# MMAThijssen/catfish

Measured on AMD Instinct MI355X. Metric: signal samples/s classified, higher is better.
Workload: dtype f32

## Files before the change

catfish_amd/csrc/catfish_hip.hip:

```cpp
#include <hip/hip_runtime.h>
#include <stdint.h>
#include <string.h>
#include <stdio.h>
#include <vector>
#include <string>
#include <cmath>
#include <mutex>
#include <set>
#include <functional>

#include "../../include/catfish_hip.h"

typedef float f32x4 __attribute__((ext_vector_type(4)));
typedef float f32x2 __attribute__((ext_vector_type(2)));

#define CF_T 35
#define CF_H 64
#define CF_C 32
#define CF_TILE 16

#define MFMA16(a, b, c) __builtin_amdgcn_mfma_f32_16x16x4f32((a), (b), (c), 0, 0, 0)

#ifndef CF_ABLATE
#define CF_ABLATE 0
// ... 52 lines not shown
__device__ __forceinline__ uint32_t cf_fmix32(uint32_t v) {
    v ^= v >> 16; v *= 0x85ebca6bu; v ^= v >> 13; v *= 0xc2b2ae35u; v ^= v >> 16;
    return v;
}
__device__ __forceinline__ uint32_t cf_drop_key(const cf_dropout& d) {
    const uint32_t st = d.step ? (uint32_t)(long long)d.step[0] : 0u;
    return cf_fmix32(d.seed ^ cf_fmix32(0x9E3779B9u * (uint32_t)(d.layer + 1) + st * 0x85ebca6bu));
}
__device__ __forceinline__ f32x4 cf_drop_scale4(uint32_t key, float keep_prob, int64_t idx4) {
    const uint32_t thresh = (uint32_t)fminf(keep_prob * 4294967296.0f, 4294967040.0f);
    const float inv = 1.0f / keep_prob;
    const uint64_t e = (uint64_t)idx4 * 4u;
    const uint32_t base = (uint32_t)e ^ ((uint32_t)(e >> 32) * 0x9E3779B9u);
    f32x4 o;
    o.x = cf_fmix32((base + 0u) ^ key) < thresh ? inv : 0.f;
    o.y = cf_fmix32((base + 1u) ^ key) < thresh ? inv : 0.f;
    o.z = cf_fmix32((base + 2u) ^ key) < thresh ? inv : 0.f;
    o.w = cf_fmix32((base + 3u) ^ key) < thresh ? inv : 0.f;
    return o;
}

__device__ __forceinline__ f32x4 relu4(f32x4 v) {
    f32x4 o;
    o.x = fmaxf(v.x, 0.f); o.y = fmaxf(v.y, 0.f); o.z = fmaxf(v.z, 0.f); o.w = fmaxf(v.w, 0.f);
    return o;
}

__host__ __device__ constexpr int gru_x_floats(int cin) { return (cin / 4) * 3 * 256; }
__host__ __device__ constexpr int gru_hg_floats() { return 16 * 2 * 256; }
__host__ __device__ constexpr int gru_hc_floats() { return 16 * 256; }
__host__ __device__ constexpr int gru_bias_off(int cin) { return gru_x_floats(cin) + gru_hg_floats() + gru_hc_floats(); }
__host__ __device__ constexpr int gru_dense_off(int cin) { return gru_bias_off(cin) + 192; }
__host__ __device__ constexpr int gru_pack_floats(int cin) { return gru_dense_off(cin) + 64; }

__host__ __device__ constexpr int res_units(bool first) { return first ? 4 : 6; }
__host__ __device__ constexpr int res_vecs(bool first) { return first ? 6 : 4; }
__host__ __device__ constexpr int res_pack_floats(bool first) { return res_units(first) * 1024 + res_vecs(first) * 32; }

__host__ __device__ constexpr int frag_feature(int ks, int q) { return 16 * (ks >> 2) + 4 * q + (ks & 3); }

__device__ __forceinline__ void unit_mma(const float* __restrict__ unit, int lane, const f32x4 (&in)[2], f32x4 (&acc)[2]) {
    const f32x2* u2 = reinterpret_cast<const f32x2*>(unit) + lane;
#pragma unroll
    for (int ks = 0; ks < 8; ++ks) {
        const f32x2 a = u2[ks * 64];
        const float b = in[ks >> 2][ks & 3];
        acc[0] = MFMA16(a.x, b, acc[0]);
        acc[1] = MFMA16(a.y, b, acc[1]);
    }
}

template <bool FIRST>
__global__ __launch_bounds__(256) void res_block_kernel(const float* __restrict__ wpack,
                                                        const float* __restrict__ x_nat,
                                                        const f32x4* __restrict__ x_frag,
                                                        f32x4* __restrict__ y_frag,
                                                        int64_t n_windows, int n_tiles, int t_chunks) {
    extern __shared__ __attribute__((aligned(16))) float lds[];
    constexpr int PACK = res_pack_floats(FIRST);
    constexpr int VEC0 = res_units(FIRST) * 1024;
    {
        const f32x4* src = reinterpret_cast<const f32x4*>(wpack);
        f32x4* dst = reinterpret_cast<f32x4*>(lds);
        for (int i = threadIdx.x; i < PACK / 4; i += blockDim.x) dst[i] = src[i];
    }
    __syncthreads();
// ... 168 lines not shown
            }
#pragma unroll
            for (int mo = 0; mo < 2; ++mo) {
                a_pp[mo] = a_p[mo]; a_p[mo] = a_c[mo]; a_sp[mo] = a_sc[mo];
                if (i >= 1) { b_pp[mo] = b_p[mo]; b_p[mo] = b_c[mo]; b_sp[mo] = b_sc[mo]; }
            }
        }
        __builtin_amdgcn_wave_barrier();
    }
}

template <int CIN>
__device__ __forceinline__ void gru_stage_weights(float* lds, const float* __restrict__ wpack, int dir) {
    constexpr int PACK = gru_pack_floats(CIN);
    const f32x4* src = reinterpret_cast<const f32x4*>(wpack + (size_t)dir * PACK);
    f32x4* dst = reinterpret_cast<f32x4*>(lds);
    for (int i = threadIdx.x; i < PACK / 4; i += blockDim.x) dst[i] = src[i];
}

#ifndef CF_SCHED_DS_FIRST
#define CF_SCHED_DS_FIRST 1
#endif
#if CF_SCHED_DS_FIRST
#define CF_KSTEP_SCHED(nds, nmfma)                               \
    __builtin_amdgcn_sched_group_barrier(0x100, nds, 0);         \
    __builtin_amdgcn_sched_group_barrier(0x008, nmfma, 0);       \
    __builtin_amdgcn_sched_barrier(0)
#else
#define CF_KSTEP_SCHED(nds, nmfma) __builtin_amdgcn_sched_barrier(0)
#endif
template <int CIN, bool LAST, bool STASH = false>
__device__ __forceinline__ void gru_tile(const float* lds, int lane, int dir, int tile, const f32x4* __restrict__ X,
                                         f32x4* __restrict__ Y, float* __restrict__ P, int n_tiles,
                                         f32x4* __restrict__ S = nullptr, f32x4* __restrict__ YD = nullptr, cf_dropout drop = cf_dropout()) {
    const uint32_t drop_key = (STASH && YD) ? cf_drop_key(drop) : 0u;
    constexpr int KGX = CIN / 16;
    constexpr int KSX = CIN / 4;
    constexpr int XN4 = gru_x_floats(CIN) / 4;
    constexpr int HG4 = gru_hg_floats() / 4;
    constexpr int BIAS = gru_bias_off(CIN);
    constexpr int DENSE = gru_dense_off(CIN);
    const int q = lane >> 4;
    const f32x4* WX = reinterpret_cast<const f32x4*>(lds) + lane;
    const far_lds<f32x4> WL(WX);
    const f32x4* B4 = reinterpret_cast<const f32x4*>(lds + BIAS) + q;
    const f32x4* D4 = reinterpret_cast<const f32x4*>(lds + DENSE) + q;
    {
        f32x4 h[4] = {{0, 0, 0, 0}, {0, 0, 0, 0}, {0, 0, 0, 0}, {0, 0, 0, 0}};
        f32x4 xc[KGX];
        {
            const int t0 = dir ? (CF_T - 1) : 0;
            const f32x4* src = X + ((int64_t)tile * CF_T + t0) * KGX * 64 + lane;
#pragma unroll
            for (int g = 0; g < KGX; ++g) xc[g] = src[g * 64];
        }
        for (int s = 0; s < CF_T; ++s) {
            const int t = dir ? (CF_T - 1 - s) : s;
            f32x4 acc[12];
#pragma unroll
            for (int mo = 0; mo < 12; ++mo) acc[mo] = B4[mo * 4];
            constexpr int PF = CF_PREFETCH;
            auto loadA = [&](int p, f32x4 (&d)[3]) {
                if (p < KSX) { d[0] = WL[(p * 3 + 0) * 64]; d[1] = WL[(p * 3 + 1) * 64]; d[2] = WL[(p * 3 + 2) * 64]; }
                else if (p < KSX + 16) { d[0] = WL[XN4 + ((p - KSX) * 2 + 0) * 64]; d[1] = WL[XN4 + ((p - KSX) * 2 + 1) * 64]; }
                else if (p < KSX + 32) { d[0] = WL[XN4 + HG4 + (p - KSX - 16) * 64]; }
            };
            f32x4 ac[3], an[3], a2[3];
            loadA(0, ac);
            if (PF == 2) loadA(1, an);
#pragma unroll
            for (int ks = 0; ks < KSX; ++ks) {
                if (PF == 2) loadA(ks + 2, a2); else loadA(ks + 1, an);
                const float b = xc[ks >> 2][ks & 3];
#pragma unroll
                for (int g = 0; g < 3; ++g) {
                    acc[4 * g + 0] = MFMA16(ac[g].x, b, acc[4 * g + 0]);
                    acc[4 * g + 1] = MFMA16(ac[g].y, b, acc[4 * g + 1]);
                    acc[4 * g + 2] = MFMA16(ac[g].z, b, acc[4 * g + 2]);
                    acc[4 * g + 3] = MFMA16(ac[g].w, b, acc[4 * g + 3]);
                }
                CF_KSTEP_SCHED(3, 12);
#pragma unroll
                for (int g = 0; g < 3; ++g) { ac[g] = an[g]; if (PF == 2) an[g] = a2[g]; }
            }
            {
                int tn = dir ? (t - 1) : (t + 1);
                tn = tn < 0 ? 0 : (tn > CF_T - 1 ? CF_T - 1 : tn);
                const f32x4* src = X + ((int64_t)tile * CF_T + tn) * KGX * 64 + lane;
#pragma unroll
// ... 43 lines not shown
                if constexpr (STASH) { acc[4 + m] = u; acc[8 + m] = c; }
            }
            if constexpr (STASH) {
                f32x4* sdst = S + (((int64_t)tile * CF_T + t) * 2 + dir) * 12 * 64 + lane;
#pragma unroll
                for (int j = 0; j < 12; ++j) sdst[j * 64] = acc[j];
            }
            if constexpr (!LAST) {
                f32x4* dst = Y + (((int64_t)tile * CF_T + t) * 8 + dir * 4) * 64 + lane;
#pragma unroll
                for (int m = 0; m < 4; ++m) if (!(CF_ABLATE & 2) || s == CF_T - 1) dst[m * 64] = h[m];
                if constexpr (STASH) {
                    if (YD) {
                        const int64_t i0 = (((int64_t)tile * CF_T + t) * 8 + dir * 4) * 64 + lane;
#pragma unroll
                        for (int m = 0; m < 4; ++m) YD[i0 + m * 64] = h[m] * cf_drop_scale4(drop_key, drop.keep_prob, i0 + m * 64);
                    }
                }
            } else {
                float pm[4];
#pragma unroll
                for (int m = 0; m < 4; ++m) {
                    const f32x4 wd = D4[m * 4];
                    pm[m] = wd.x * h[m].x;
                    pm[m] = fmaf(wd.y, h[m].y, pm[m]); pm[m] = fmaf(wd.z, h[m].z, pm[m]); pm[m] = fmaf(wd.w, h[m].w, pm[m]);
                }
                float p = ((pm[0] + pm[1]) + pm[2]) + pm[3];
                p += __shfl_xor(p, 16);
                p += __shfl_xor(p, 32);
                if (lane < 16) P[(((int64_t)dir * n_tiles + tile) * CF_T + t) * 16 + lane] = p;
            }
            __builtin_amdgcn_sched_barrier(0);
        }
    }
}

template <int CIN, bool LAST>
__global__ __launch_bounds__(512, 2) void gru_layer_kernel(const float* __restrict__ wpack,
                                                           const f32x4* __restrict__ X,
                                                           f32x4* __restrict__ Y,
                                                           float* __restrict__ P,
                                                           int n_tiles) {
    extern __shared__ __attribute__((aligned(16))) float lds[];
    const int dir = blockIdx.y;
    gru_stage_weights<CIN>(lds, wpack, dir);
    __syncthreads();
    const int lane = threadIdx.x & 63;
    const int wave = __builtin_amdgcn_readfirstlane(threadIdx.x >> 6);
    const int nwaves = blockDim.x >> 6;
    const int t0 = (int)((int64_t)blockIdx.x * n_tiles / gridDim.x);
    const int t1 = (int)((int64_t)(blockIdx.x + 1) * n_tiles / gridDim.x);
    for (int tile = t0 + wave; tile < t1; tile += nwaves)
        gru_tile<CIN, LAST>(lds, lane, dir, tile, X, Y, P, n_tiles);
}

struct cf_fused_args {
    const float* w[3];
    const f32x4* x0;
    f32x4* y[2];
    float* p;
    unsigned* flags;
    int lds_floats;
    unsigned* err;
    int n_tiles;
    int groups;
    int n_layers;
    int cin0;
};

__device__ __forceinline__ bool cf_wait_flag(unsigned* flag) {
    for (int it = 0; it < 1000000; ++it) {
        if (__hip_atomic_load(flag, __ATOMIC_RELAXED, __HIP_MEMORY_SCOPE_AGENT) != 0u) return true;
        __builtin_amdgcn_s_sleep(16);
    }
    return false;
}

template <int CIN, bool LAST>
__device__ __forceinline__ void gru_fused_worker(float* lds, const cf_fused_args& a, int layer, int dir) {
    const f32x4* X = layer == 0 ? a.x0 : a.y[(layer - 1) & 1];
    f32x4* Y = a.y[layer & 1];
    gru_stage_weights<CIN>(lds, a.w[layer], dir);
    volatile int* slot = reinterpret_cast<volatile int*>(lds + a.lds_floats);
    unsigned* queue = a.flags + (size_t)a.n_layers * a.groups * 2 + layer * 2 + dir;
    const int lane = threadIdx.x & 63;
    const int wave = __builtin_amdgcn_readfirstlane(threadIdx.x >> 6);
// ... 270 lines not shown
    do {                                                                                           \
        hipError_t e_ = (expr);                                                                    \
        if (e_ != hipSuccess)                                                                      \
            return fail(CF_ERR_HIP, std::string(#expr) + ": " + hipGetErrorString(e_));           \
    } while (0)

enum { SLOT_RES_FIRST = 0, SLOT_RES, SLOT_GRU0, SLOT_GRU, SLOT_GRU_LAST, SLOT_HEAD, SLOT_POST, SLOT_NORM, SLOT_GRU_FUSED, SLOT_RES_STACK2 };
static const char* k_slot_names[CF_PROF_SLOTS] = {"res_block_first", "res_block",      "gru_layer_first", "gru_layer_mid",
                                                  "gru_layer_last",  "head",           "postprocess",     "normalize",       "gru_fused",
                                                  "res_stack2",      "unused",         "unused"};

struct cf_param_map;
static void pm_destroy(cf_param_map* pm);

struct cf_model {
    cf_hparams hp;
    int device = 0;
    int n_cu = 256;
    std::vector<float*> d_res;
    std::vector<float*> d_gru;
    std::vector<int> gru_cin;
    std::vector<char*> d_res_b;
    std::vector<char*> d_gru_b;
    int np = 0;
    float* d_dense_bias = nullptr;
    cf_param_map* pmap = nullptr;
    int64_t cap_windows = 0;
    int64_t cap_tiles = 0;
    struct Slot {
        float* d_a[2] = {nullptr, nullptr};
        float* d_y[2] = {nullptr, nullptr};
        float* d_p = nullptr;
        unsigned* d_flags = nullptr;
        hipStream_t stream = nullptr;
        hipEvent_t done = nullptr;
        int64_t last_windows = 0;
        bool last_res_fused = false;
    };
    std::vector<Slot> slots;
    cf_generic* gen = nullptr;
    int fuse = 0;
    float* d_xp = nullptr;
    int xp_tiles = 0;
    float* d_host_x = nullptr;
    float* d_host_p = nullptr;
    size_t host_stage_bytes = 0;
    unsigned* h_err = nullptr;
    unsigned* d_err = nullptr;
    hipEvent_t fork = nullptr;
    int64_t ws_bytes = 0;
    bool prof = false;
    int prof_every = 0;
    int64_t prof_calls = 0;
    struct Ev { hipEvent_t a, b; int slot; };
    std::vector<Ev> ev_pending;
    std::vector<hipEvent_t> ev_pool;
    double prof_ms[CF_PROF_SLOTS] = {0};
    int64_t prof_n[CF_PROF_SLOTS] = {0};
};

enum { CF_TERM_ZERO = 0, CF_TERM_RAW = 1, CF_TERM_KERN = 2, CF_TERM_BIAS = 3 };
enum { CF_K_ONE = 0, CF_K_GATE = 1, CF_K_CAND = 2 };
__host__ __device__ inline double cf_term_const(int c) { return c == CF_K_GATE ? CF_GATE_SCALE : (c == CF_K_CAND ? CF_CAND_SCALE : 1.0); }

__host__ __device__ inline double cf_bn_scale(float gamma, float var, float eps) {
#pragma clang fp contract(off)
// ... 207 lines not shown
    const size_t pd = off + gru_dense_off(cin);
    for (int i = 0; i < CF_H; ++i) e(pd + i, dense_t >= 0 ? cf_raw(dense_t, dense_e + i) : cf_zero());
}

static void pack_gru_dir(const cf_gru_dir& g, int cin, int cin_real, const float* dense_w ,
                         float* out) {
    cf_host_params P;
    P.t = {g.gates_kernel, g.gates_bias, g.candidate_kernel, g.candidate_bias, dense_w};
    HostSink e{P, out};
    pack_gru_dir(e, 0, gru_terms(0, CF_H), cin, cin_real, dense_w ? 4 : -1, 0);
}

static int upload(const std::vector<float>& host, float** dev) {
    HIP_TRY(hipMalloc((void**)dev, host.size() * sizeof(float)));
    HIP_TRY(hipMemcpy(*dev, host.data(), host.size() * sizeof(float), hipMemcpyHostToDevice));
    return CF_OK;
}

static bool gen_wanted(const cf_hparams* hp);
static int gen_build(cf_model* m, const cf_weights* w);
static void gen_destroy(cf_generic* g);

extern "C" void cf_model_destroy(cf_model* m) {
    if (!m) return;
    (void)hipSetDevice(m->device);
    for (float* p : m->d_res) if (p) (void)hipFree(p);
    for (float* p : m->d_gru) if (p) (void)hipFree(p);
    for (char* p : m->d_gru_b) if (p) (void)hipFree(p);
    for (char* p : m->d_res_b) if (p) (void)hipFree(p);
    for (auto& sl : m->slots) {
        for (int i = 0; i < 2; ++i) { if (sl.d_a[i]) (void)hipFree(sl.d_a[i]); if (sl.d_y[i]) (void)hipFree(sl.d_y[i]); }
        if (sl.d_p) (void)hipFree(sl.d_p);
        if (sl.d_flags) (void)hipFree(sl.d_flags);
        if (sl.stream) (void)hipStreamDestroy(sl.stream);
        if (sl.done) (void)hipEventDestroy(sl.done);
    }
    gen_destroy(m->gen);
    pm_destroy(m->pmap);
    if (m->d_dense_bias) (void)hipFree(m->d_dense_bias);
    if (m->d_xp) (void)hipFree(m->d_xp);
    if (m->d_host_x) (void)hipFree(m->d_host_x);
    if (m->h_err) (void)hipHostFree(m->h_err);
    if (m->fork) (void)hipEventDestroy(m->fork);
    for (auto& e : m->ev_pending) { (void)hipEventDestroy(e.a); (void)hipEventDestroy(e.b); }
    for (auto& e : m->ev_pool) (void)hipEventDestroy(e);
    delete m;
}

extern "C" int cf_model_create(const cf_weights* w, const cf_hparams* hp, int device, cf_model** out) {
    if (!w || !hp || !out) return fail(CF_ERR_INVALID, "cf_model_create: null argument");
    *out = nullptr;
    if (hp->window != CF_T) return fail(CF_ERR_INVALID, "window must be 35 (rnn_class.py:27)");
    if (hp->n_layers < 1 || hp->n_layers_res < 0) return fail(CF_ERR_INVALID, "n_layers must be >= 1 and n_layers_res >= 0");
    const bool generic = gen_wanted(hp);
    if (!generic && hp->n_layers_res == 0 && hp->precision != CF_PREC_FP32)
        return fail(CF_ERR_INVALID, "the plain RNN type (n_layers_res = 0) is only built for CF_PREC_FP32");
    if ((hp->n_layers_res > 0 && !w->conv) || !w->gru || !w->dense_kernel || !w->dense_bias)
        return fail(CF_ERR_INVALID, "cf_weights has null members");
    int n_dev = 0;
    HIP_TRY(hipGetDeviceCount(&n_dev));
    if (device < 0 || device >= n_dev) return fail(CF_ERR_INVALID, "device index out of range");
    HIP_TRY(hipSetDevice(device));

    if (hp->precision < CF_PREC_FP32 || hp->precision > CF_PREC_BF16)
        return fail(CF_ERR_INVALID, "precision must be CF_PREC_FP32, CF_PREC_BF16X3 or CF_PREC_BF16");
    cf_model* m = new cf_model();
// ... 38 lines not shown
        const int cin_real = l == 0 ? (hp->n_layers_res > 0 ? CF_C : 1) : 2 * CF_H;
        const int cin = cin_real == 1 ? 16 : cin_real;
        if (w->gru[2 * l].cin != cin_real || w->gru[2 * l + 1].cin != cin_real) { rc = fail(CF_ERR_INVALID, "GRU layer input width mismatch"); break; }
        const bool last = l == hp->n_layers - 1;
        std::vector<float> blob((size_t)2 * gru_pack_floats(cin));
        HostSink e{P, blob.data()};
        for (int d = 0; d < 2; ++d)
            pack_gru_dir(e, (size_t)d * gru_pack_floats(cin), gru_terms(cf_tid_gru(hp->n_layers_res, l, d, 0), CF_H), cin, cin_real,
                         last ? cf_tid_dense(hp->n_layers_res, hp->n_layers, 0) : -1, d * CF_H);
        float* dptr = nullptr;
        rc = upload(blob, &dptr);
        m->d_gru.push_back(dptr);
        m->gru_cin.push_back(cin);
        if (rc == CF_OK && m->np > 0) {
            const size_t bytes = (size_t)gb_pack_bytes(cin, m->np);
            std::vector<char> bblob(2 * bytes, 0);
            for (int d = 0; d < 2; ++d)
                pack_gru_dir_bf16(w->gru[2 * l + d], cin, m->np, last ? w->dense_kernel + d * CF_H : nullptr, bblob.data() + d * bytes);
            char* bptr = nullptr;
            hipError_t e = hipMalloc((void**)&bptr, bblob.size());
            if (e == hipSuccess) e = hipMemcpy(bptr, bblob.data(), bblob.size(), hipMemcpyHostToDevice);
            if (e != hipSuccess) rc = fail(CF_ERR_HIP, std::string("bf16 weight upload: ") + hipGetErrorString(e));
            m->d_gru_b.push_back(bptr);
        }
    }
    if (rc == CF_OK) {
        int64_t cap = hp->max_windows_per_pass > 0 ? hp->max_windows_per_pass : 32768;
        cap = (cap + 2 * CF_TILE - 1) / (2 * CF_TILE) * (2 * CF_TILE);
        m->cap_windows = cap;
        m->cap_tiles = cap / CF_TILE;
        const size_t a_bytes = (size_t)m->cap_tiles * CF_T * 2 * 64 * sizeof(f32x4);
        const size_t y_bytes = (size_t)m->cap_tiles * CF_T * 8 * 64 * sizeof(f32x4);
        const size_t p_bytes = std::max((size_t)2 * m->cap_tiles * CF_T * 16, (size_t)2 * std::min<int64_t>(m->cap_tiles, m->n_cu) * CF_T * 256) * sizeof(float);
        hipError_t e = hipSuccess;
        int n_slots = hp->n_streams > 0 ? hp->n_streams : 1;
        if (n_slots > 8) n_slots = 8;
        m->slots.resize(n_slots);
        for (auto& sl : m->slots) {
            for (int i = 0; i < 2 && e == hipSuccess; ++i) e = hipMalloc((void**)&sl.d_a[i], a_bytes);
            for (int i = 0; i < 2 && e == hipSuccess; ++i) e = hipMalloc((void**)&sl.d_y[i], y_bytes);
            if (e == hipSuccess) e = hipMalloc((void**)&sl.d_p, p_bytes);
            if (e == hipSuccess) e = hipMalloc((void**)&sl.d_flags, (size_t)3 * ((m->cap_tiles + 7) / 8) * 2 * sizeof(unsigned) + 64);
            if (e == hipSuccess && n_slots > 1) e = hipStreamCreateWithFlags(&sl.stream, hipStreamNonBlocking);
            if (e == hipSuccess && n_slots > 1) e = hipEventCreateWithFlags(&sl.done, hipEventDisableTiming);
        }
        if (e == hipSuccess && n_slots > 1) e = hipEventCreateWithFlags(&m->fork, hipEventDisableTiming);
        if (e == hipSuccess && n_slots == 1 && m->np == 0) {
            int xpt = (int)std::min<int64_t>(m->cap_tiles, std::max(1, 3 * m->n_cu / 16));
            if (cf_knob("CATFISH_HOIST_TILES")) xpt = std::max(1, std::min(atoi(cf_knob("CATFISH_HOIST_TILES")), (int)m->cap_tiles));
            e = hipMalloc((void**)&m->d_xp, (size_t)xpt * CF_T * 2 * 12 * 64 * sizeof(f32x4));
            if (e == hipSuccess) m->xp_tiles = xpt;
        }
        if (e == hipSuccess) e = hipHostMalloc((void**)&m->h_err, sizeof(unsigned), hipHostMallocMapped);
        if (e == hipSuccess) { *m->h_err = 0u; e = hipHostGetDevicePointer((void**)&m->d_err, m->h_err, 0); }
        m->fuse = (m->np == 0 && hp->n_layers <= 3 && hp->fuse_layers >= 0) ? (hp->fuse_layers > 0 ? 1 : 2) : 0;
        if (cf_knob("CATFISH_FUSE") && m->fuse) m->fuse = atoi(cf_knob("CATFISH_FUSE")) != 0 ? 1 : 0;
        if (e != hipSuccess) rc = fail(CF_ERR_NOMEM, std::string("workspace allocation: ") + hipGetErrorString(e));
        m->ws_bytes = (int64_t)n_slots * (int64_t)(2 * a_bytes + 2 * y_bytes + p_bytes);
    }
    if (rc == CF_OK) {
        hipError_t e = hipSuccess;
        auto optin = [&](const void* f, int bytes) { if (e == hipSuccess) e = hipFuncSetAttribute(f, hipFuncAttributeMaxDynamicSharedMemorySize, bytes); };
        optin((const void*)gru_layer_kernel<16, false>, gru_pack_floats(16) * 4);
        optin((const void*)gru_layer_kernel<16, true>, gru_pack_floats(16) * 4);
        optin((const void*)gru_layer_kernel<32, false>, gru_pack_floats(32) * 4);
        optin((const void*)gru_layer_kernel<32, true>, gru_pack_floats(32) * 4);
        optin((const void*)gru_layer_kernel<128, false>, gru_pack_floats(128) * 4);
        optin((const void*)gru_layer_kernel<128, true>, gru_pack_floats(128) * 4);
        optin((const void*)gru_fused_kernel, gru_pack_floats(128) * 4 + 16);
        optin((const void*)gru_layer_coop_kernel<16, false>, (gru_pack_floats(16) + CF_COOP_XCH_FLOATS) * 4);
        optin((const void*)gru_layer_coop_kernel<16, true>, (gru_pack_floats(16) + CF_COOP_XCH_FLOATS) * 4);
        optin((const void*)gru_layer_coop_kernel<32, false>, (gru_pack_floats(32) + CF_COOP_XCH_FLOATS) * 4);
        optin((const void*)gru_layer_coop_kernel<32, true>, (gru_pack_floats(32) + CF_COOP_XCH_FLOATS) * 4);
        optin((const void*)gru_layer_coop_kernel<128, false>, (gru_pack_floats(128) + CF_COOP_XCH_FLOATS) * 4);
        optin((const void*)gru_layer_coop_kernel<128, true>, (gru_pack_floats(128) + CF_COOP_XCH_FLOATS) * 4);
        optin((const void*)gru_train_fwd_coop_kernel<32>, (gru_pack_floats(32) + CF_COOP_XCH_FLOATS) * 4);
        optin((const void*)gru_train_fwd_coop_kernel<128>, (gru_pack_floats(128) + CF_COOP_XCH_FLOATS) * 4);
        optin((const void*)gru_train_bwd_coop_kernel<32>, (gtb_pack_floats(32) + CF_COOP_BWD_XCH_FLOATS) * 4);
        optin((const void*)gru_train_bwd_coop_kernel<128>, (gtb_pack_floats(128) + CF_COOP_BWD_XCH_FLOATS) * 4);
        optin((const void*)gru_train_fwd_kernel<32>, gru_pack_floats(32) * 4);
        optin((const void*)gru_train_fwd_kernel<128>, gru_pack_floats(128) * 4);
        optin((const void*)gru_train_bwd_kernel<32>, gtb_pack_floats(32) * 4);
        optin((const void*)gru_train_bwd_kernel<128>, gtb_pack_floats(128) * 4);
        optin((const void*)res_stack2_kernel<true>, (res_pack_floats(true) + res_pack_floats(false) + 4 * CF_TILE * CF_T) * 4);
        optin((const void*)res_stack2_kernel<false>, (res_pack_floats(true) + res_pack_floats(false) + 4 * CF_TILE * CF_T) * 4);
        optin((const void*)res_train_fwd_kernel, RT_FWD_LDS_BYTES);
        optin((const void*)res_train_bwd_kernel, RT_BWD_LDS_BYTES);
        optin((const void*)gru_layer_bf16_kernel<32, false, 1>, gb_pack_bytes(32, 1));
        optin((const void*)gru_layer_bf16_kernel<32, true, 1>, gb_pack_bytes(32, 1));
        optin((const void*)gru_layer_bf16_kernel<128, false, 1>, gb_pack_bytes(128, 1));
        optin((const void*)gru_layer_bf16_kernel<128, true, 1>, gb_pack_bytes(128, 1));
        optin((const void*)gru_bf16_pipe_kernel<32, false>, gb_pack_bytes(32, 1));
        optin((const void*)gru_bf16_pipe_kernel<32, true>, gb_pack_bytes(32, 1));
        optin((const void*)gru_bf16_pipe_kernel<128, false>, gb_pack_bytes(128, 1));
        optin((const void*)gru_bf16_pipe_kernel<128, true>, gb_pack_bytes(128, 1));
        optin((const void*)gru_xproj_lds_kernel<32>, gru_x_floats(32) * 4);
        optin((const void*)gru_xproj_lds_kernel<128>, gru_x_floats(128) * 4);
        optin((const void*)gru_bf16x3_pipe_kernel<32, false>, gb_pack_bytes(32, 2));
        optin((const void*)gru_bf16x3_pipe_kernel<32, true>, gb_pack_bytes(32, 2));
        optin((const void*)gru_bf16x3_pipe_kernel<128, false>, gb_pack_bytes(128, 2));
        optin((const void*)gru_bf16x3_pipe_kernel<128, true>, gb_pack_bytes(128, 2));
// ... 27 lines not shown
    return CF_OK;
}

static int pick_waves(int n_tile_tasks, int n_cu) {
    int w = (n_tile_tasks + n_cu - 1) / n_cu;
    return w <= 1 ? 1 : (w <= 2 ? 2 : (w <= 4 ? 4 : 8));
}

static bool use_coop(const cf_model* m, int n_tiles) {
    static const int coop_env = cf_knob("CATFISH_COOP") ? atoi(cf_knob("CATFISH_COOP")) : -1;
    const bool coop = coop_env >= 0 ? coop_env != 0 : n_tiles <= m->n_cu;
    return coop && !(CF_ABLATE & 4) && n_tiles <= m->n_cu;
}

template <int CIN>
static void launch_xproj(cf_model* m, const float* wpack, const float* X, int n_tiles, hipStream_t s) {
    const int lds_env = cf_knob("CATFISH_XPROJ_LDS") ? atoi(cf_knob("CATFISH_XPROJ_LDS")) : 1;
    if (lds_env) {
        int chunks = cf_xproj_plan(n_tiles, m->n_cu, CIN);
        if (cf_knob("CATFISH_XPROJ_CHUNKS")) {
            const int c = std::max(1, std::min(CF_T, atoi(cf_knob("CATFISH_XPROJ_CHUNKS"))));
            const int tl = (CF_T + c - 1) / c;
            chunks = (CF_T + tl - 1) / tl;
        }
        hipLaunchKernelGGL((gru_xproj_lds_kernel<CIN>), dim3(n_tiles * chunks, 2), dim3(256), gru_x_floats(CIN) * 4, s, wpack,
                           reinterpret_cast<const f32x4*>(X), reinterpret_cast<f32x4*>(m->d_xp), n_tiles, chunks);
    } else {
        hipLaunchKernelGGL((gru_xproj_kernel<CIN>), dim3(n_tiles * cf_xproj_chunks(n_tiles), 2), dim3(256), 0, s, wpack,
                           reinterpret_cast<const f32x4*>(X), reinterpret_cast<f32x4*>(m->d_xp), n_tiles, cf_xproj_chunks(n_tiles));
    }
}

template <int CIN, bool LAST>
static int launch_gru(cf_model* m, const float* wpack, const float* X, float* Y, float* P, int n_tiles, hipStream_t s, int slot) {
    if (use_coop(m, n_tiles)) {
        size_t pi = 0;
        int rc = prof_begin(m, slot, s, &pi);
        if (rc != CF_OK) return rc;
        const int gx = std::min(n_tiles, std::max(1, m->n_cu / 2));
        const f32x4* xp = nullptr;
        if (CIN >= 32 && n_tiles <= m->xp_tiles) {
            xp = reinterpret_cast<const f32x4*>(m->d_xp);
            launch_xproj<CIN>(m, wpack, X, n_tiles, s);
        }
        hipLaunchKernelGGL((gru_layer_coop_kernel<CIN, LAST>), dim3(gx, 2), dim3(256), (gru_pack_floats(CIN) + CF_COOP_XCH_FLOATS) * 4, s,
                           wpack, reinterpret_cast<const f32x4*>(X), reinterpret_cast<f32x4*>(Y), P, n_tiles, xp);
        HIP_TRY(hipGetLastError());
        return prof_end(m, s, pi);
    }
    static const int waves_env = cf_knob("CATFISH_WAVES") ? atoi(cf_knob("CATFISH_WAVES")) : 0;
    const int waves = waves_env > 0 ? std::min(waves_env, 8) : ((CF_ABLATE & 4) ? 4 : pick_waves(2 * n_tiles, m->n_cu));
    const int groups = (n_tiles + waves - 1) / waves;
    int per_dir = m->n_cu / 2 > 0 ? m->n_cu / 2 : 1;
    constexpr int lds_bytes = gru_pack_floats(CIN) * 4;
    if (lds_bytes <= 80 * 1024) per_dir *= 2;
    const int gx = groups < per_dir ? groups : per_dir;
    size_t pi = 0;
    int rc = prof_begin(m, slot, s, &pi);
    if (rc != CF_OK) return rc;
    hipLaunchKernelGGL((gru_layer_kernel<CIN, LAST>), dim3(gx, 2), dim3(waves * 64), lds_bytes, s, wpack,
                       reinterpret_cast<const f32x4*>(X), reinterpret_cast<f32x4*>(Y), P, n_tiles);
    HIP_TRY(hipGetLastError());
    return prof_end(m, s, pi);
}

template <int CIN, bool LAST, int NP>
static int launch_gru_bf16(cf_model* m, const char* wpack, const float* X, float* Y, float* P, int n_tiles32, hipStream_t s, int slot) {
    static const int waves_env = cf_knob("CATFISH_BF16_WAVES") ? atoi(cf_knob("CATFISH_BF16_WAVES")) : 0;
    static const int wgs_env = cf_knob("CATFISH_BF16_WGS") ? atoi(cf_knob("CATFISH_BF16_WGS")) : 0;
    const int waves = waves_env > 0 ? std::min(waves_env, 8) : pick_waves(2 * n_tiles32, m->n_cu);
    const int groups = (n_tiles32 + waves - 1) / waves;
    int per_dir = m->n_cu / 2 > 0 ? m->n_cu / 2 : 1;
    constexpr int lds_bytes = gb_pack_bytes(CIN, NP);
    if (lds_bytes <= 80 * 1024) per_dir *= 2;
    if (wgs_env > 0) per_dir = wgs_env;
    const int gx = groups < per_dir ? groups : per_dir;
    size_t pi = 0;
    int rc = prof_begin(m, slot, s, &pi);
    if (rc != CF_OK) return rc;
    const int pipe_env = cf_knob("CATFISH_BF16_PIPE") ? atoi(cf_knob("CATFISH_BF16_PIPE")) : 1;
    if constexpr (NP == 1) {
        if (pipe_env) {
            hipLaunchKernelGGL((gru_bf16_pipe_kernel<CIN, LAST>), dim3(gx, 2), dim3(waves * 64), lds_bytes, s, wpack,
                               reinterpret_cast<const bf16x8*>(X), reinterpret_cast<bf16x8*>(Y), P, n_tiles32);
            HIP_TRY(hipGetLastError());
            return prof_end(m, s, pi);
        }
    }
    if constexpr (NP == 2) {
        if (pipe_env) {
            const int w4 = std::min(waves, 4);
            const int g4 = (n_tiles32 + w4 - 1) / w4;
            const int per4 = wgs_env > 0 ? wgs_env : std::max(1, m->n_cu / 2);
            hipLaunchKernelGGL((gru_bf16x3_pipe_kernel<CIN, LAST>), dim3(std::min(g4, per4), 2), dim3(w4 * 64), lds_bytes, s, wpack,
// ... 128 lines not shown
        if ((rc = prof_end(m, s, pi)) != CF_OK) return rc;
    }
    const float* cur = m->hp.n_layers_res == 0 ? sl.d_a[0] : sl.d_a[(m->hp.n_layers_res - 1) & 1];
    const bool fuse_now = m->fuse == 1 || (m->fuse == 2 && (n_tiles + 7) / 8 >= cf_fuse_min_groups(m->n_cu));
    if (fuse_now) {
        cf_fused_args a;
        for (int l = 0; l < 3; ++l) a.w[l] = l < m->hp.n_layers ? m->d_gru[l] : nullptr;
        a.x0 = reinterpret_cast<const f32x4*>(cur);
        a.y[0] = reinterpret_cast<f32x4*>(sl.d_y[0]);
        a.y[1] = reinterpret_cast<f32x4*>(sl.d_y[1]);
        a.p = sl.d_p;
        a.flags = sl.d_flags;
        a.err = m->d_err;
        a.n_tiles = n_tiles;
        a.groups = (n_tiles + 7) / 8;
        a.n_layers = m->hp.n_layers;
        a.cin0 = m->hp.n_layers_res == 0 ? 16 : CF_C;
        HIP_TRY(hipMemsetAsync(sl.d_flags, 0, ((size_t)a.n_layers * a.groups * 2 + (size_t)a.n_layers * 2) * sizeof(unsigned), s));
        if ((rc = prof_begin(m, SLOT_GRU_FUSED, s, &pi)) != CF_OK) return rc;
        a.lds_floats = m->hp.n_layers > 1 ? gru_pack_floats(128) : gru_pack_floats(a.cin0);
        const int lds_bytes = a.lds_floats * 4 + 16;
        const int pool = std::min(a.groups, std::max(1, m->n_cu / 2)) * 2;
        hipLaunchKernelGGL(gru_fused_kernel, dim3((unsigned)(a.n_layers * pool)), dim3(512), lds_bytes, s, a);
        HIP_TRY(hipGetLastError());
        if ((rc = prof_end(m, s, pi)) != CF_OK) return rc;
    }
    for (int l = 0; l < (fuse_now ? 0 : m->hp.n_layers); ++l) {
        const bool last = l == m->hp.n_layers - 1;
        float* y = sl.d_y[l & 1];
        if (m->np > 0) {
            rc = m->np == 1 ? launch_gru_bf16_layer<1>(m, l, last, cur, y, sl.d_p, n_tiles32, s)
                            : launch_gru_bf16_layer<2>(m, l, last, cur, y, sl.d_p, n_tiles32, s);
        } else if (l == 0 && m->hp.n_layers_res == 0) {
            rc = last ? launch_gru<16, true>(m, m->d_gru[l], cur, y, sl.d_p, n_tiles, s, SLOT_GRU_LAST)
                      : launch_gru<16, false>(m, m->d_gru[l], cur, y, sl.d_p, n_tiles, s, SLOT_GRU0);
        } else if (l == 0) {
            rc = last ? launch_gru<32, true>(m, m->d_gru[l], cur, y, sl.d_p, n_tiles, s, SLOT_GRU_LAST)
                      : launch_gru<32, false>(m, m->d_gru[l], cur, y, sl.d_p, n_tiles, s, SLOT_GRU0);
        } else {
            rc = last ? launch_gru<128, true>(m, m->d_gru[l], cur, y, sl.d_p, n_tiles, s, SLOT_GRU_LAST)
                      : launch_gru<128, false>(m, m->d_gru[l], cur, y, sl.d_p, n_tiles, s, SLOT_GRU);
        }
        if (rc != CF_OK) return rc;
        cur = y;
    }
    if ((rc = prof_begin(m, SLOT_HEAD, s, &pi)) != CF_OK) return rc;
    const int64_t total = n_windows * CF_T;
    const int raw_partials = (m->np == 0 && !fuse_now && use_coop(m, n_tiles)) ? 1 : 0;
    hipLaunchKernelGGL(head_kernel, dim3((unsigned)((total + 255) / 256)), dim3(256), 0, s, sl.d_p, m->d_dense_bias, probs, logits, n_windows,
                       m->np > 0 ? n_tiles32 : n_tiles, m->np > 0 ? 5 : 4, raw_partials);
    HIP_TRY(hipGetLastError());
    if ((rc = prof_end(m, s, pi)) != CF_OK) return rc;
    sl.last_windows = n_windows;
    return CF_OK;
}

static const char* k_fused_timeout_msg = "a fused biGRU launch timed out waiting for a producer workgroup; its results are invalid "
                                         "(create the model with fuse_layers = -1)";

extern "C" int cf_check_error(cf_model* m) {
    if (!m) return fail(CF_ERR_INVALID, "cf_check_error: null model");
    if (m->h_err && *m->h_err) return fail(CF_ERR_HIP, k_fused_timeout_msg);
    return CF_OK;
}

extern "C" int cf_clear_error(cf_model* m) {
    if (!m) return fail(CF_ERR_INVALID, "cf_clear_error: null model");
    if (m->h_err) *m->h_err = 0u;
    return CF_OK;
}

extern "C" int cf_launch_regimes(const cf_model* m, int64_t out[4]) {
    if (!m || !out) return fail(CF_ERR_INVALID, "cf_launch_regimes: null argument");
    out[0] = m->n_cu;
// ... 703 lines not shown
```

Before: 325.8 million.

## Balance GRU timesteps across waves with split-tile hidden-state handoff

```diff
diff --git a/catfish_amd/csrc/catfish_hip.hip b/catfish_amd/csrc/catfish_hip.hip
--- a/catfish_amd/csrc/catfish_hip.hip
+++ b/catfish_amd/csrc/catfish_hip.hip
@@ -108,6 +108,8 @@
 __host__ __device__ constexpr int gru_bias_off(int cin) { return gru_x_floats(cin) + gru_hg_floats() + gru_hc_floats(); }
 __host__ __device__ constexpr int gru_dense_off(int cin) { return gru_bias_off(cin) + 192; }
 __host__ __device__ constexpr int gru_pack_floats(int cin) { return gru_dense_off(cin) + 64; }
+#define CF_GRU_MAX_WAVES 8
+#include "gru_balance.hpp"
 
 __host__ __device__ constexpr int res_units(bool first) { return first ? 4 : 6; }
 __host__ __device__ constexpr int res_vecs(bool first) { return first ? 6 : 4; }
@@ -342,7 +344,8 @@
 template <int CIN, bool LAST, bool STASH = false>
 __device__ __forceinline__ void gru_tile(const float* lds, int lane, int dir, int tile, const f32x4* __restrict__ X,
                                          f32x4* __restrict__ Y, float* __restrict__ P, int n_tiles,
-                                         f32x4* __restrict__ S = nullptr, f32x4* __restrict__ YD = nullptr, cf_dropout drop = cf_dropout()) {
+                                         f32x4* __restrict__ S = nullptr, f32x4* __restrict__ YD = nullptr, cf_dropout drop = cf_dropout(),
+                                         int s_begin = 0, int s_end = CF_T, f32x4* HO = nullptr) {
     const uint32_t drop_key = (STASH && YD) ? cf_drop_key(drop) : 0u;
     constexpr int KGX = CIN / 16;
     constexpr int KSX = CIN / 4;
@@ -357,14 +360,18 @@
     const f32x4* D4 = reinterpret_cast<const f32x4*>(lds + DENSE) + q;
     {
         f32x4 h[4] = {{0, 0, 0, 0}, {0, 0, 0, 0}, {0, 0, 0, 0}, {0, 0, 0, 0}};
+        if (s_begin > 0) {
+#pragma unroll
+            for (int m = 0; m < 4; ++m) h[m] = HO[m * 64 + lane];
+        }
         f32x4 xc[KGX];
         {
-            const int t0 = dir ? (CF_T - 1) : 0;
+            const int t0 = dir ? (CF_T - 1 - s_begin) : s_begin;
             const f32x4* src = X + ((int64_t)tile * CF_T + t0) * KGX * 64 + lane;
 #pragma unroll
             for (int g = 0; g < KGX; ++g) xc[g] = src[g * 64];
         }
-        for (int s = 0; s < CF_T; ++s) {
+        for (int s = s_begin; s < s_end; ++s) {
             const int t = dir ? (CF_T - 1 - s) : s;
             f32x4 acc[12];
 #pragma unroll
@@ -474,7 +481,30 @@
             }
             __builtin_amdgcn_sched_barrier(0);
         }
-    }
+        if (s_end < CF_T) {
+#pragma unroll
+            for (int m = 0; m < 4; ++m) HO[m * 64 + lane] = h[m];
+        }
+    }
+}
+
+__device__ __forceinline__ void cf_handoff_publish(unsigned* flag) {
+    asm volatile("s_waitcnt vmcnt(0)" ::: "memory");
+    __builtin_amdgcn_fence(__ATOMIC_RELEASE, "workgroup");
+    asm volatile("s_waitcnt vmcnt(0)" ::: "memory");
+    __hip_atomic_store(flag, 1u, __ATOMIC_RELAXED, __HIP_MEMORY_SCOPE_WORKGROUP);
+}
+__device__ __forceinline__ void cf_handoff_wait(unsigned* flag, int lane, unsigned* err) {
+    if (lane == 0) {
+        bool ok = false;
+        for (int it = 0; it < 1000000 && !ok; ++it) {
+            ok = __hip_atomic_load(flag, __ATOMIC_RELAXED, __HIP_MEMORY_SCOPE_WORKGROUP) != 0u;
+            if (!ok) __builtin_amdgcn_s_sleep(16);
+        }
+        if (!ok && err) __hip_atomic_store(err, 1u, __ATOMIC_RELAXED, __HIP_MEMORY_SCOPE_SYSTEM);
+    }
+    __builtin_amdgcn_fence(__ATOMIC_ACQUIRE, "workgroup");
+    asm volatile("s_waitcnt vmcnt(0)" ::: "memory");
 }
 
 template <int CIN, bool LAST>
@@ -482,18 +512,48 @@
                                                            const f32x4* __restrict__ X,
                                                            f32x4* __restrict__ Y,
                                                            float* __restrict__ P,
-                                                           int n_tiles) {
+                                                           int n_tiles,
+                                                           int balance,
+                                                           f32x4* hand,
+                                                           unsigned* err) {
     extern __shared__ __attribute__((aligned(16))) float lds[];
     const int dir = blockIdx.y;
     gru_stage_weights<CIN>(lds, wpack, dir);
+    unsigned* flags = reinterpret_cast<unsigned*>(lds + gru_pack_floats(CIN));
+    if (threadIdx.x < CF_GRU_MAX_WAVES) flags[threadIdx.x] = 0u;
     __syncthreads();
     const int lane = threadIdx.x & 63;
     const int wave = __builtin_amdgcn_readfirstlane(threadIdx.x >> 6);
     const int nwaves = blockDim.x >> 6;
     const int t0 = (int)((int64_t)blockIdx.x * n_tiles / gridDim.x);
     const int t1 = (int)((int64_t)(blockIdx.x + 1) * n_tiles / gridDim.x);
-    for (int tile = t0 + wave; tile < t1; tile += nwaves)
-        gru_tile<CIN, LAST>(lds, lane, dir, tile, X, Y, P, n_tiles);
+    cf_gru_share sh;
+    int n_pieces;
+    if (balance) {
+        sh = cf_gru_balanced_share(t1 - t0, nwaves, wave, CF_T);
+        n_pieces = (sh.head_end > 0) + sh.whole_count + (sh.tail_begin < CF_T);
+    } else {
+        sh.head_tile = sh.head_end = 0; sh.whole_first = sh.whole_count = 0; sh.tail_tile = 0; sh.tail_begin = CF_T;
+        n_pieces = t1 - t0 > wave ? (t1 - t0 - wave + nwaves - 1) / nwaves : 0;
+    }
+    f32x4* slots = hand + ((size_t)(dir * gridDim.x + blockIdx.x) * CF_GRU_MAX_WAVES) * 4 * 64;
+    const int has_head = balance && sh.head_end > 0;
+    for (int i = 0; i < n_pieces; ++i) {
+        int tile, s_begin = 0, s_end = CF_T;
+        f32x4* ho = nullptr;
+        if (!balance) {
+            tile = t0 + wave + i * nwaves;
+        } else if (i < has_head) {
+            tile = t0 + sh.head_tile; s_end = sh.head_end; ho = slots + wave * 4 * 64;
+        } else if (i < has_head + sh.whole_count) {
+            tile = t0 + sh.whole_first + (i - has_head);
+        } else {
+            tile = t0 + sh.tail_tile; s_begin = sh.tail_begin; ho = slots + (wave - 1) * 4 * 64;
+            cf_handoff_wait(flags + (wave - 1), lane, err);
+        }
+        gru_tile<CIN, LAST>(lds, lane, dir, tile, X, Y, P, n_tiles, nullptr, nullptr, cf_dropout(), s_begin, s_end, ho);
+        if (s_end < CF_T) cf_handoff_publish(flags + wave);
+    }
 }
 
 struct cf_fused_args {
@@ -830,6 +890,7 @@
         float* d_y[2] = {nullptr, nullptr};
         float* d_p = nullptr;
         unsigned* d_flags = nullptr;
+        float* d_hand = nullptr;
         hipStream_t stream = nullptr;
         hipEvent_t done = nullptr;
         int64_t last_windows = 0;
@@ -1103,6 +1164,7 @@
         for (int i = 0; i < 2; ++i) { if (sl.d_a[i]) (void)hipFree(sl.d_a[i]); if (sl.d_y[i]) (void)hipFree(sl.d_y[i]); }
         if (sl.d_p) (void)hipFree(sl.d_p);
         if (sl.d_flags) (void)hipFree(sl.d_flags);
+        if (sl.d_hand) (void)hipFree(sl.d_hand);
         if (sl.stream) (void)hipStreamDestroy(sl.stream);
         if (sl.done) (void)hipEventDestroy(sl.done);
     }
@@ -1207,6 +1269,7 @@
         const size_t a_bytes = (size_t)m->cap_tiles * CF_T * 2 * 64 * sizeof(f32x4);
         const size_t y_bytes = (size_t)m->cap_tiles * CF_T * 8 * 64 * sizeof(f32x4);
         const size_t p_bytes = std::max((size_t)2 * m->cap_tiles * CF_T * 16, (size_t)2 * std::min<int64_t>(m->cap_tiles, m->n_cu) * CF_T * 256) * sizeof(float);
+        const size_t hand_bytes = (size_t)2 * (2 * std::max(1, m->n_cu / 2)) * CF_GRU_MAX_WAVES * 4 * 64 * sizeof(f32x4);
         hipError_t e = hipSuccess;
         int n_slots = hp->n_streams > 0 ? hp->n_streams : 1;
         if (n_slots > 8) n_slots = 8;
@@ -1216,6 +1279,7 @@
             for (int i = 0; i < 2 && e == hipSuccess; ++i) e = hipMalloc((void**)&sl.d_y[i], y_bytes);
             if (e == hipSuccess) e = hipMalloc((void**)&sl.d_p, p_bytes);
             if (e == hipSuccess) e = hipMalloc((void**)&sl.d_flags, (size_t)3 * ((m->cap_tiles + 7) / 8) * 2 * sizeof(unsigned) + 64);
+            if (e == hipSuccess && m->np == 0) e = hipMalloc((void**)&sl.d_hand, hand_bytes);
             if (e == hipSuccess && n_slots > 1) e = hipStreamCreateWithFlags(&sl.stream, hipStreamNonBlocking);
             if (e == hipSuccess && n_slots > 1) e = hipEventCreateWithFlags(&sl.done, hipEventDisableTiming);
         }
@@ -1231,17 +1295,17 @@
         m->fuse = (m->np == 0 && hp->n_layers <= 3 && hp->fuse_layers >= 0) ? (hp->fuse_layers > 0 ? 1 : 2) : 0;
         if (cf_knob("CATFISH_FUSE") && m->fuse) m->fuse = atoi(cf_knob("CATFISH_FUSE")) != 0 ? 1 : 0;
         if (e != hipSuccess) rc = fail(CF_ERR_NOMEM, std::string("workspace allocation: ") + hipGetErrorString(e));
-        m->ws_bytes = (int64_t)n_slots * (int64_t)(2 * a_bytes + 2 * y_bytes + p_bytes);
+        m->ws_bytes = (int64_t)n_slots * (int64_t)(2 * a_bytes + 2 * y_bytes + p_bytes + (m->np == 0 ? hand_bytes : 0));
     }
     if (rc == CF_OK) {
         hipError_t e = hipSuccess;
         auto optin = [&](const void* f, int bytes) { if (e == hipSuccess) e = hipFuncSetAttribute(f, hipFuncAttributeMaxDynamicSharedMemorySize, bytes); };
-        optin((const void*)gru_layer_kernel<16, false>, gru_pack_floats(16) * 4);
-        optin((const void*)gru_layer_kernel<16, true>, gru_pack_floats(16) * 4);
-        optin((const void*)gru_layer_kernel<32, false>, gru_pack_floats(32) * 4);
-        optin((const void*)gru_layer_kernel<32, true>, gru_pack_floats(32) * 4);
-        optin((const void*)gru_layer_kernel<128, false>, gru_pack_floats(128) * 4);
-        optin((const void*)gru_layer_kernel<128, true>, gru_pack_floats(128) * 4);
+        optin((const void*)gru_layer_kernel<16, false>, gru_pack_floats(16) * 4 + CF_GRU_MAX_WAVES * 4);
+        optin((const void*)gru_layer_kernel<16, true>, gru_pack_floats(16) * 4 + CF_GRU_MAX_WAVES * 4);
+        optin((const void*)gru_layer_kernel<32, false>, gru_pack_floats(32) * 4 + CF_GRU_MAX_WAVES * 4);
+        optin((const void*)gru_layer_kernel<32, true>, gru_pack_floats(32) * 4 + CF_GRU_MAX_WAVES * 4);
+        optin((const void*)gru_layer_kernel<128, false>, gru_pack_floats(128) * 4 + CF_GRU_MAX_WAVES * 4);
+        optin((const void*)gru_layer_kernel<128, true>, gru_pack_floats(128) * 4 + CF_GRU_MAX_WAVES * 4);
         optin((const void*)gru_fused_kernel, gru_pack_floats(128) * 4 + 16);
         optin((const void*)gru_layer_coop_kernel<16, false>, (gru_pack_floats(16) + CF_COOP_XCH_FLOATS) * 4);
         optin((const void*)gru_layer_coop_kernel<16, true>, (gru_pack_floats(16) + CF_COOP_XCH_FLOATS) * 4);
@@ -1335,7 +1399,8 @@
 }
 
 template <int CIN, bool LAST>
-static int launch_gru(cf_model* m, const float* wpack, const float* X, float* Y, float* P, int n_tiles, hipStream_t s, int slot) {
+static int launch_gru(cf_model* m, const float* wpack, const float* X, float* Y, float* P, int n_tiles, hipStream_t s, int slot,
+                      float* hand = nullptr) {
     if (use_coop(m, n_tiles)) {
         size_t pi = 0;
         int rc = prof_begin(m, slot, s, &pi);
@@ -1357,12 +1422,26 @@
     int per_dir = m->n_cu / 2 > 0 ? m->n_cu / 2 : 1;
     constexpr int lds_bytes = gru_pack_floats(CIN) * 4;
     if (lds_bytes <= 80 * 1024) per_dir *= 2;
-    const int gx = groups < per_dir ? groups : per_dir;
+    int gx = groups < per_dir ? groups : per_dir;
     size_t pi = 0;
     int rc = prof_begin(m, slot, s, &pi);
     if (rc != CF_OK) return rc;
-    hipLaunchKernelGGL((gru_layer_kernel<CIN, LAST>), dim3(gx, 2), dim3(waves * 64), lds_bytes, s, wpack,
-                       reinterpret_cast<const f32x4*>(X), reinterpret_cast<f32x4*>(Y), P, n_tiles);
+    int balance = 0;
+    if (hand) {
+        const int wg_per_cu = std::max(1, (2 * gx + m->n_cu - 1) / m->n_cu);
+        const int gx_one = std::max(1, m->n_cu / 2);
+        const int load_rr = cf_gru_grid_load(n_tiles, gx, waves, wg_per_cu, CF_T, 0);
+        const int load_bal = cf_gru_grid_load(n_tiles, gx, waves, wg_per_cu, CF_T, 1);
+        const int load_one = gx > gx_one ? cf_gru_grid_load(n_tiles, gx_one, waves, 1, CF_T, 1) : -1;
+        const char* env = cf_knob("CATFISH_GRU_BALANCE");
+        const int forced = env ? atoi(env) : -1;
+        int best = load_rr;
+        if (forced < 0 ? (load_bal >= 0 && load_bal < best) : (forced >= 1 && load_bal >= 0)) { balance = 1; best = load_bal; }
+        if (forced < 0 ? (load_one >= 0 && load_one < best) : (forced == 2 && load_one >= 0)) { balance = 1; gx = gx_one; }
+    }
+    hipLaunchKernelGGL((gru_layer_kernel<CIN, LAST>), dim3(gx, 2), dim3(waves * 64), lds_bytes + CF_GRU_MAX_WAVES * 4, s, wpack,
+                       reinterpret_cast<const f32x4*>(X), reinterpret_cast<f32x4*>(Y), P, n_tiles, balance, reinterpret_cast<f32x4*>(hand),
+                       m->d_err);
     HIP_TRY(hipGetLastError());
     return prof_end(m, s, pi);
 }
@@ -1557,14 +1636,14 @@
             rc = m->np == 1 ? launch_gru_bf16_layer<1>(m, l, last, cur, y, sl.d_p, n_tiles32, s)
                             : launch_gru_bf16_layer<2>(m, l, last, cur, y, sl.d_p, n_tiles32, s);
         } else if (l == 0 && m->hp.n_layers_res == 0) {
-            rc = last ? launch_gru<16, true>(m, m->d_gru[l], cur, y, sl.d_p, n_tiles, s, SLOT_GRU_LAST)
-                      : launch_gru<16, false>(m, m->d_gru[l], cur, y, sl.d_p, n_tiles, s, SLOT_GRU0);
+            rc = last ? launch_gru<16, true>(m, m->d_gru[l], cur, y, sl.d_p, n_tiles, s, SLOT_GRU_LAST, sl.d_hand)
+                      : launch_gru<16, false>(m, m->d_gru[l], cur, y, sl.d_p, n_tiles, s, SLOT_GRU0, sl.d_hand);
         } else if (l == 0) {
-            rc = last ? launch_gru<32, true>(m, m->d_gru[l], cur, y, sl.d_p, n_tiles, s, SLOT_GRU_LAST)
-                      : launch_gru<32, false>(m, m->d_gru[l], cur, y, sl.d_p, n_tiles, s, SLOT_GRU0);
+            rc = last ? launch_gru<32, true>(m, m->d_gru[l], cur, y, sl.d_p, n_tiles, s, SLOT_GRU_LAST, sl.d_hand)
+                      : launch_gru<32, false>(m, m->d_gru[l], cur, y, sl.d_p, n_tiles, s, SLOT_GRU0, sl.d_hand);
         } else {
-            rc = last ? launch_gru<128, true>(m, m->d_gru[l], cur, y, sl.d_p, n_tiles, s, SLOT_GRU_LAST)
-                      : launch_gru<128, false>(m, m->d_gru[l], cur, y, sl.d_p, n_tiles, s, SLOT_GRU);
+            rc = last ? launch_gru<128, true>(m, m->d_gru[l], cur, y, sl.d_p, n_tiles, s, SLOT_GRU_LAST, sl.d_hand)
+                      : launch_gru<128, false>(m, m->d_gru[l], cur, y, sl.d_p, n_tiles, s, SLOT_GRU, sl.d_hand);
         }
         if (rc != CF_OK) return rc;
         cur = y;
diff --git a/catfish_amd/csrc/gru_balance.hpp b/catfish_amd/csrc/gru_balance.hpp
--- /dev/null
+++ b/catfish_amd/csrc/gru_balance.hpp
@@ -0,0 +1,67 @@
+#pragma once
+
+#if defined(__HIPCC__) || defined(__CUDACC__)
+#define CF_BAL_HD __host__ __device__
+#else
+#define CF_BAL_HD
+#endif
+
+struct cf_gru_share {
+    int head_tile, head_end;
+    int whole_first, whole_count;
+    int tail_tile, tail_begin;
+    int interior;
+    int steps;
+};
+
+CF_BAL_HD inline cf_gru_share cf_gru_balanced_share(int tiles, int nwaves, int wave, int T) {
+    const int total = tiles * T;
+    const int a = (int)((long long)wave * total / nwaves), b = (int)((long long)(wave + 1) * total / nwaves);
+    cf_gru_share s;
+    s.steps = b - a;
+    s.tail_tile = a / T;
+    s.tail_begin = a % T == 0 ? T : a % T;
+    s.head_tile = b / T;
+    s.head_end = b % T;
+    s.interior = (a % T != 0 && b % T != 0 && a / T == b / T) ? 1 : 0;
+    s.whole_first = (a + T - 1) / T;
+    s.whole_count = b / T - s.whole_first;
+    if (s.whole_count < 0) s.whole_count = 0;
+    return s;
+}
+
+CF_BAL_HD inline int cf_gru_round_robin_steps(int tiles, int nwaves, int wave, int T) {
+    return wave < tiles ? ((tiles - wave + nwaves - 1) / nwaves) * T : 0;
+}
+
+CF_BAL_HD inline bool cf_gru_balance_ok(int tiles, int nwaves, int T) {
+    if (tiles < 1 || nwaves < 1) return false;
+    for (int w = 0; w < nwaves; ++w) {
+        const cf_gru_share s = cf_gru_balanced_share(tiles, nwaves, w, T);
+        if (s.interior || s.steps <= 0) return false;
+    }
+    return true;
+}
+
+CF_BAL_HD inline int cf_gru_simd_load(int tiles, int nwaves, int T, int balanced) {
+    const int per_simd = (nwaves + 3) / 4;
+    int top[2] = {0, 0};
+    for (int w = 0; w < nwaves; ++w) {
+        int v = balanced ? cf_gru_balanced_share(tiles, nwaves, w, T).steps : cf_gru_round_robin_steps(tiles, nwaves, w, T);
+        if (v > top[0]) { const int t = top[0]; top[0] = v; v = t; }
+        if (v > top[1]) top[1] = v;
+    }
+    return per_simd >= 2 ? top[0] + top[1] : top[0];
+}
+
+CF_BAL_HD inline int cf_gru_grid_load(int n_tiles, int gx, int nwaves, int wg_per_cu, int T, int balanced) {
+    if (gx < 1 || n_tiles < gx) return balanced ? -1 : cf_gru_simd_load(1, nwaves, T, 0) * wg_per_cu;
+    const int lo = n_tiles / gx, hi = (n_tiles % gx) ? lo + 1 : lo;
+    int worst = 0;
+    for (int t = lo; t <= hi; ++t) {
+        if (balanced && !cf_gru_balance_ok(t, nwaves, T)) return -1;
+        const int v = cf_gru_simd_load(t, nwaves, T, balanced);
+        if (v > worst) worst = v;
+    }
+    return worst * wg_per_cu;
+}
```

New measurement: 340.6 million, median of 6. 4.6% higher.
